# vovw/algonauts-2025

Measured on AMD Instinct MI355X. Metric: TRs/sec trimodal encode to 1000 parcels, higher is better.
Workload: dtype bf16; 1 GPU; trimodal encode, precomputed bf16 feats, per GPU B=64 sequences (4 subjects x R=16) x T=1024, L*D=4096 per modality, hidden 3072, 8 layers, V=1000 parcels, n_output_timesteps=1024; forward only; global_batch=64, seq_len=1024, parallelism=dp1

## Files before the change

algonauts-2025_amd/csrc/attention.hip:

```cpp
#include "attn_common.h"
#include "attn_acc_regs.h"

namespace {

template <int DH>
struct AttnCfg {
  static constexpr int NSUB = DH <= 64 ? 4 : (DH <= 128 ? 2 : 1);
  static constexpr int KS = DH / 32;
  static constexpr int DT = DH / 16;
  static constexpr int ROWB = DH * 2;
  static constexpr int KV = 32 * NSUB;
  static constexpr int TILE_BYTES = KV * ROWB;
  static constexpr int CHUNKS = DH / 8;
  static constexpr int WAVES = 8;
  static constexpr int PIECES = KV * CHUNKS / 64;
  static constexpr int PPW = (PIECES + WAVES - 1) / WAVES;
  static constexpr int SWZ_MASK = (CHUNKS % 16 == 0) ? 15 : 7;
  static constexpr int NBUF = DH >= 192 ? 3 : 2;
  static constexpr int SMEM = NBUF * 2 * TILE_BYTES;
  static_assert(DH % 64 == 0, "dim_head must be a multiple of 64");
};

template <int DH>
__device__ __forceinline__ int swz_chunk(int chunk, int row) {
  constexpr int MASK = AttnCfg<DH>::SWZ_MASK;
  return (chunk & ~MASK) | ((chunk ^ ((row & 7) << 1)) & MASK);
}


template <int DH, int CAUSAL, int RELKEY>
__global__ __launch_bounds__(512, 2) void attn_fwd_kernel(const AttnArgs a) {
  using C = AttnCfg<DH>;
  extern __shared__ __attribute__((aligned(16))) char smem[];
  const int tid = threadIdx.x, lane = tid & 63;
  const int wave = __builtin_amdgcn_readfirstlane(tid >> 6);
  const int fq = lane >> 4, l15 = lane & 15;

  const int T = a.T;
  const float scale_log2e = a.scale_log2e;
  const int xcd = blockIdx.x & 7, slot = blockIdx.x >> 3;
  const int qb = slot % a.qblocks;
  const int pair = (slot / a.qblocks) * 8 + xcd;
  if (pair >= a.n_bh) return;
  const int h = pair % a.heads_q;
  const int b = pair / a.heads_q;
  const int hk = h / a.group;
  const int64_t ld = a.ld_kv;
  const unsigned short* qbase = a.q + (int64_t)b * T * a.ld_q + (int64_t)h * DH;
  const unsigned short* kbase = a.k + (int64_t)b * T * ld + (int64_t)hk * DH;
  const unsigned short* vbase = a.v + (int64_t)b * T * ld + (int64_t)hk * DH;

  const int q0 = qb * 128 + wave * 16;
  const int qrow = (q0 + l15 < T) ? q0 + l15 : T - 1;
  bf16x8_t qf[C::KS];
#pragma unroll
  for (int ks = 0; ks < C::KS; ++ks) qf[ks] = *(const bf16x8_t*)(qbase + (int64_t)qrow * a.ld_q + ks * 32 + fq * 8);

  int st_row[C::PPW], st_src[C::PPW], st_off[C::PPW];
#pragma unroll
  for (int i = 0; i < C::PPW; ++i) {
    const int p = (wave + C::WAVES * i) * 64 + lane;
    st_row[i] = p / C::CHUNKS;
    st_src[i] = swz_chunk<DH>(p % C::CHUNKS, st_row[i]) * 8;
    st_off[i] = st_row[i] * (int)ld + st_src[i];
  }
  auto stage = [&](int buf, int key0) {
    char* kdst = smem + buf * 2 * C::TILE_BYTES;
    const unsigned short* kb = kbase + (int64_t)key0 * ld;
    const unsigned short* vb = vbase + (int64_t)key0 * ld;
    const bool full = key0 + C::KV <= T;
#pragma unroll
    for (int i = 0; i < C::PPW; ++i) {
      const int piece = wave + C::WAVES * i;
      if (piece < C::PIECES) {
        int off = st_off[i];
        if (!full) {
          const int row = (key0 + st_row[i] < T) ? st_row[i] : T - 1 - key0;
          off = row * (int)ld + st_src[i];
        }
        glds16(kb + off, lds_addr(kdst + piece * 1024));
        glds16(vb + off, lds_addr(kdst + C::TILE_BYTES + piece * 1024));
      }
    }
  };

  constexpr int SEG = C::SWZ_MASK + 1;
  constexpr int KRD = SEG / 4;
  int k_rd[KRD];
#pragma unroll
  for (int i = 0; i < KRD; ++i) k_rd[i] = l15 * C::ROWB + swz_chunk<DH>(4 * i + fq, l15) * 16;
  const int tq = l15 >> 2, tp = l15 & 3;
  constexpr int VRD = SEG / 2;
  int v_rd[VRD];
#pragma unroll
  for (int i = 0; i < VRD; ++i) {
    const int row = 4 * fq + tq;
    v_rd[i] = row * C::ROWB + swz_chunk<DH>(2 * i + (tp >> 1), row) * 16 + (tp & 1) * 8;
  }

  f32x4_t o[C::DT];
#pragma unroll
  for (int dt = 0; dt < C::DT; ++dt) o[dt] = f32x4_t{0.f, 0.f, 0.f, 0.f};
  float m_run = -INFINITY, l_run = 0.f;
  constexpr bool LSUM_MFMA = C::NSUB > 1;
  f32x4_t lacc = {0.f, 0.f, 0.f, 0.f};
  bf16x8_t ones;
#pragma unroll
  for (int e = 0; e < 8; ++e) ones[e] = (short)0x3F80;

  int kv_end = T;
  if (CAUSAL) { const int last_q = qb * 128 + 127; kv_end = (last_q + 1 < T) ? last_q + 1 : T; }
  const int ntiles = (kv_end + C::KV - 1) / C::KV;
  int my_glds = 0;
#pragma unroll
  for (int i = 0; i < C::PPW; ++i) my_glds += (wave + C::WAVES * i < C::PIECES) ? 2 : 0;
  auto wait_keep_one_tile = [&]() {
    if (my_glds >= 6) asm volatile("s_waitcnt vmcnt(6)" ::: "memory");
    else if (my_glds == 4) asm volatile("s_waitcnt vmcnt(4)" ::: "memory");
    else if (my_glds == 2) asm volatile("s_waitcnt vmcnt(2)" ::: "memory");
    else asm volatile("s_waitcnt vmcnt(0)" ::: "memory");
  };
  static_assert(C::NBUF == 2 || C::PPW <= 3, "wait_keep_one_tile handles up to 6 loads per tile and wave");
  stage(0, 0);
  if (C::NBUF == 3 && ntiles > 1) { stage(1, C::KV); wait_keep_one_tile(); } else { asm volatile("s_waitcnt vmcnt(0)" ::: "memory"); }
  __syncthreads();

  for (int t = 0; t < ntiles; ++t) {
    const int cur = t % C::NBUF;
    if (C::NBUF == 2 && t + 1 < ntiles) stage(cur ^ 1, (t + 1) * C::KV);
    const char* kt = smem + cur * 2 * C::TILE_BYTES;
    const char* vt = kt + C::TILE_BYTES;
    if (!CAUSAL || t * C::KV <= q0 + 15) {

    float sv[C::NSUB][8];
    float pmax = -INFINITY;
    const int lim = CAUSAL ? ((q0 + l15 + 1 < T) ? q0 + l15 + 1 : T) : T;
#pragma unroll
    for (int u = 0; u < C::NSUB; ++u) {
      const int sub_key0 = t * C::KV + u * 32;
      if (sub_key0 >= T || (CAUSAL && sub_key0 > q0 + 15)) {
#pragma unroll
        for (int j = 0; j < 8; ++j) sv[u][j] = -INFINITY;
        continue;
      }
      f32x4_t s0 = {0.f, 0.f, 0.f, 0.f}, s1 = {0.f, 0.f, 0.f, 0.f};
#pragma unroll
      for (int ks = 0; ks < C::KS; ++ks) {
        const int off = k_rd[ks % KRD] + (ks / KRD) * SEG * 16 + u * 32 * C::ROWB;
        const bf16x8_t ka = *(const bf16x8_t*)(kt + off);
        const bf16x8_t kb2 = *(const bf16x8_t*)(kt + off + 16 * C::ROWB);
        s0 = __builtin_amdgcn_mfma_f32_16x16x32_bf16(ka, qf[ks], s0, 0, 0, 0);
        s1 = __builtin_amdgcn_mfma_f32_16x16x32_bf16(kb2, qf[ks], s1, 0, 0, 0);
      }
      const int key_base = sub_key0 + 4 * fq;
      if (RELKEY) {
        const float* qrow_e = a.qe + ((int64_t)b * T + qrow) * a.ld_qe + h * a.qe_stride_h + a.rel_left;
#pragma unroll
        for (int r = 0; r < 4; ++r) {
          int d0 = key_base + r - qrow, d1 = key_base + 16 + r - qrow;
          d0 = d0 < -a.rel_left ? -a.rel_left : (d0 > a.rel_right ? a.rel_right : d0);
          d1 = d1 < -a.rel_left ? -a.rel_left : (d1 > a.rel_right ? a.rel_right : d1);
          s0[r] += qrow_e[d0];
          s1[r] += qrow_e[d1];
        }
      }
      const bool edge = sub_key0 + 32 > T || (CAUSAL && sub_key0 + 31 > q0);
      if (edge) {
#pragma unroll
        for (int r = 0; r < 4; ++r) {
          sv[u][r] = (key_base + r < lim) ? s0[r] : -INFINITY;
          sv[u][4 + r] = (key_base + 16 + r < lim) ? s1[r] : -INFINITY;
        }
      } else {
#pragma unroll
        for (int r = 0; r < 4; ++r) { sv[u][r] = s0[r]; sv[u][4 + r] = s1[r]; }
      }
      pmax = fmaxf(pmax, fmaxf(sv[u][0], sv[u][4]));
#pragma unroll
      for (int r = 1; r < 4; ++r) pmax = max3f(pmax, sv[u][r], sv[u][4 + r]);
    }
    pmax = fmaxf(pmax, __shfl_xor(pmax, 16, 64));
    pmax = fmaxf(pmax, __shfl_xor(pmax, 32, 64));
    pmax *= scale_log2e;
    if (!__all(pmax - m_run <= 8.0f)) {
      const float m_new = fmaxf(m_run, pmax);
      const float alpha = __builtin_amdgcn_exp2f(m_run - m_new);
      m_run = m_new;
      l_run *= alpha;
      if (LSUM_MFMA) {
#pragma unroll
        for (int r = 0; r < 4; ++r) lacc[r] *= alpha;
      }
#pragma unroll
      for (int dt = 0; dt < C::DT; ++dt)
#pragma unroll
        for (int r = 0; r < 4; ++r) o[dt][r] *= alpha;
    }
    bf16x8_t pf[C::NSUB];
    float psum = 0.f;
#pragma unroll
    for (int u = 0; u < C::NSUB; ++u)
#pragma unroll
      for (int j = 0; j < 8; ++j) {
        const float p = __builtin_amdgcn_exp2f(fmaf(sv[u][j], scale_log2e, -m_run));
        if (!LSUM_MFMA) psum += p;
        pf[u][j] = (short)f32_to_bf16(p);
      }
    l_run += psum;

#pragma unroll
    for (int u = 0; u < C::NSUB; ++u) {
      const int sub_key0 = t * C::KV + u * 32;
      if (sub_key0 >= T || (CAUSAL && sub_key0 > q0 + 15)) continue;
      if (LSUM_MFMA) lacc = __builtin_amdgcn_mfma_f32_16x16x32_bf16(ones, pf[u], lacc, 0, 0, 0);
#pragma unroll
      for (int dt = 0; dt < C::DT; ++dt) {
        const int off = v_rd[dt % VRD] + (dt / VRD) * SEG * 16 + u * 32 * C::ROWB;
        const s16x4_t lo = __builtin_amdgcn_ds_read_tr16_b64_v4i16((__attribute__((address_space(3))) s16x4_t*)(vt + off));
        const s16x4_t hi =
            __builtin_amdgcn_ds_read_tr16_b64_v4i16((__attribute__((address_space(3))) s16x4_t*)(vt + off + 16 * C::ROWB));
        bf16x8_t vf;
#pragma unroll
        for (int e = 0; e < 4; ++e) { vf[e] = lo[e]; vf[4 + e] = hi[e]; }
        o[dt] = __builtin_amdgcn_mfma_f32_16x16x32_bf16(vf, pf[u], o[dt], 0, 0, 0);
      }
    }
    }
    if (C::NBUF == 3) {
      asm volatile("s_waitcnt lgkmcnt(0)" ::: "memory");
      if (t + 2 < ntiles) { stage((t + 2) % C::NBUF, (t + 2) * C::KV); wait_keep_one_tile(); }
      else { asm volatile("s_waitcnt vmcnt(0)" ::: "memory"); }
      __builtin_amdgcn_s_barrier();
    } else {
      asm volatile("s_waitcnt vmcnt(0)" ::: "memory");
      __syncthreads();
    }
  }

  float l_tot;
  if (LSUM_MFMA) {
    l_tot = lacc[0];
  } else {
    l_tot = l_run + __shfl_xor(l_run, 16, 64);
    l_tot += __shfl_xor(l_tot, 32, 64);
  }
  const float inv = 1.0f / l_tot;
  const int q = q0 + l15;
  if (q < T) {
    unsigned short* orow = a.out + ((int64_t)b * T + q) * a.ld_out + (int64_t)h * DH + 4 * fq;
#pragma unroll
    for (int dt = 0; dt < C::DT; ++dt) {
      u16x4_t pk;
#pragma unroll
      for (int e = 0; e < 4; ++e) pk[e] = f32_to_bf16(o[dt][e] * inv);
      *(u16x4_t*)(orow + 16 * dt) = pk;
    }
  }
}


struct WideCfg {
  static constexpr int DH = 384, KS = 24, DT = 12, ROWB = 768, KV = 32, CHUNKS = 48;
  static constexpr int TILE_BYTES = KV * ROWB;
  static constexpr int WAVES = 4, PPW = 6;
  static constexpr int K_SLOTS = 2, V_SLOTS = 4;
  static constexpr int V_BASE = K_SLOTS * TILE_BYTES;
  static constexpr int SMEM = (K_SLOTS + V_SLOTS) * TILE_BYTES;
  static constexpr int DEPTH = 6;
};

__device__ __forceinline__ int swz_wide(int chunk, int row) {
  return (chunk & ~15) | ((chunk ^ (((row & 3) << 2) | ((row >> 2) & 3))) & 15);
}


__device__ __forceinline__ void mfma_s_first(f32x16_t& acc, const bf16x8_t& a, const bf16x8_t& b) {
  asm volatile("v_mfma_f32_32x32x16_bf16 %0, %1, %2, 0" : "=&v"(acc) : "v"(a), "v"(b));
}
__device__ __forceinline__ void mfma_s(f32x16_t& acc, const bf16x8_t& a, const bf16x8_t& b) {
  asm volatile("v_mfma_f32_32x32x16_bf16 %0, %1, %2, %0" : "+v"(acc) : "v"(a), "v"(b));
}


__global__ __launch_bounds__(256, 1) void attn_fwd_wide384_kernel(const AttnArgs a) {
  using C = WideCfg;
  extern __shared__ __attribute__((aligned(16))) char smem[];
  const int tid = threadIdx.x, lane = tid & 63;
  const int wave = __builtin_amdgcn_readfirstlane(tid >> 6);
  const int r31 = lane & 31, h = lane >> 5;

  const int T = a.T;
  const float scale_log2e = a.scale_log2e;
  const int xcd = blockIdx.x & 7, slot = blockIdx.x >> 3;
  const int qb = slot % a.qblocks;
  const int pair = (slot / a.qblocks) * 8 + xcd;
  if (pair >= a.n_bh) return;
  const int hd = pair % a.heads_q;
  const int b = pair / a.heads_q;
  const int hk = hd / a.group;
  const int64_t ld = a.ld_kv;
  const unsigned short* qbase = a.q + (int64_t)b * T * a.ld_q + (int64_t)hd * C::DH;
  const unsigned short* kbase = a.k + (int64_t)b * T * ld + (int64_t)hk * C::DH;
  const unsigned short* vbase = a.v + (int64_t)b * T * ld + (int64_t)hk * C::DH;

  const int q0 = qb * 128 + wave * 32;
  const int qrow = (q0 + r31 < T) ? q0 + r31 : T - 1;
  bf16x8_t qf[C::KS];
#pragma unroll
  for (int ks = 0; ks < C::KS; ++ks) qf[ks] = *(const bf16x8_t*)(qbase + (int64_t)qrow * a.ld_q + ks * 16 + h * 8);
  if (a.q_cos) {
    const int half = a.q_rot_dim >> 1;
    const float* cr = a.q_cos + (int64_t)qrow * half;
    const float* sr = a.q_sin + (int64_t)qrow * half;
#pragma unroll
    for (int ks = 0; ks < C::KS; ++ks) {
      const int d0 = ks * 16 + h * 8;
      if (d0 < a.q_rot_dim) {
        const float4 c4 = *(const float4*)(cr + (d0 >> 1)), s4 = *(const float4*)(sr + (d0 >> 1));
        const float cs[4] = {c4.x, c4.y, c4.z, c4.w}, sn[4] = {s4.x, s4.y, s4.z, s4.w};
#pragma unroll
        for (int pp = 0; pp < 4; ++pp) {
          const float qa = bf16_to_f32((unsigned short)qf[ks][2 * pp]), qb = bf16_to_f32((unsigned short)qf[ks][2 * pp + 1]);
          qf[ks][2 * pp] = (short)f32_to_bf16(qa * cs[pp] - qb * sn[pp]);
          qf[ks][2 * pp + 1] = (short)f32_to_bf16(qb * cs[pp] + qa * sn[pp]);
        }
      }
    }
  }

  int st_row[C::PPW], st_src[C::PPW], st_off[C::PPW];
#pragma unroll
  for (int i = 0; i < C::PPW; ++i) {
    const int p = (wave + C::WAVES * i) * 64 + lane;
    st_row[i] = p / C::CHUNKS;
    st_src[i] = swz_wide(p % C::CHUNKS, st_row[i]) * 8;
    st_off[i] = st_row[i] * (int)ld + st_src[i];
  }
  const unsigned lds0_u = __builtin_amdgcn_readfirstlane(lds_addr(smem));
  auto stage_piece = [&](int which, int slot, int key0, int i) {
    const char* sbase = (const char*)((which ? vbase : kbase) + (int64_t)key0 * ld);
    const int piece = wave + C::WAVES * i;
    unsigned voff = (unsigned)st_off[i] * 2u;
    if (key0 + C::KV > T) {
      const int row = (key0 + st_row[i] < T) ? st_row[i] : T - 1 - key0;
      voff = (unsigned)(row * (int)ld + st_src[i]) * 2u;
    }
    const unsigned dst = lds0_u + (which ? C::V_BASE : 0) + slot * C::TILE_BYTES + piece * 1024;
    asm volatile("s_mov_b32 m0, %0\n\ts_nop 0\n\tglobal_load_lds_dwordx4 %1, %2" : : "s"(dst), "v"(voff), "s"(sbase) : "memory");
  };
  auto stage = [&](int which, int slot, int key0) {
#pragma unroll
    for (int i = 0; i < C::PPW; ++i) stage_piece(which, slot, key0, i);
  };

  int kb_off[8];
#pragma unroll
  for (int i = 0; i < 8; ++i) kb_off[i] = r31 * C::ROWB + swz_wide(2 * i + h, r31) * 16;
  const int tq = (lane & 15) >> 2, tp = lane & 3, g1 = (lane >> 4) & 1;
  int vb_off[4][2];
#pragma unroll
  for (int i = 0; i < 4; ++i)
#pragma unroll
    for (int lh = 0; lh < 2; ++lh) {
      const int row = 4 * h + tq + 8 * lh;
      vb_off[i][lh] = C::V_BASE + row * C::ROWB + swz_wide(4 * i + 2 * g1 + (tp >> 1), row) * 16 + (tp & 1) * 8;
    }
  auto ld_k = [&](const int (&ka)[8], int ks) -> bf16x8_t {
    return *(const bf16x8_t*)(smem + ka[ks & 7] + (ks >> 3) * 256);
  };
  auto ld_v = [&](const int (&va)[4][2], int i) -> bf16x8_t {
    const int s = i / C::DT, dt = i % C::DT;
    const int imm = (dt >> 2) * 256 + s * 16 * C::ROWB;
    const s16x4_t lo = __builtin_amdgcn_ds_read_tr16_b64_v4i16((__attribute__((address_space(3))) s16x4_t*)(smem + va[dt & 3][0] + imm));
    const s16x4_t hi = __builtin_amdgcn_ds_read_tr16_b64_v4i16((__attribute__((address_space(3))) s16x4_t*)(smem + va[dt & 3][1] + imm));
    bf16x8_t vf;
#pragma unroll
    for (int e = 0; e < 4; ++e) { vf[e] = lo[e]; vf[4 + e] = hi[e]; }
    return vf;
  };

  static_for<0, C::DT>([&](auto dt) { AccTile<decltype(dt)::value>::zero(); });
  float m_run = -INFINITY, l_run = 0.f;

  const int ntiles = (T + C::KV - 1) / C::KV;
  stage(0, 0, 0); stage(1, 0, 0);
  if (ntiles > 1) { stage(0, 1, C::KV); stage(1, 1, C::KV); asm volatile("s_waitcnt vmcnt(12)" ::: "memory"); }
  else { asm volatile("s_waitcnt vmcnt(0)" ::: "memory"); }
  __builtin_amdgcn_s_barrier();

  bf16x8_t kf[C::KS], vf[2 * C::DT];
  int ka[8], va[4][2];
#pragma unroll
  for (int i = 0; i < 8; ++i) ka[i] = kb_off[i];
#pragma unroll
  for (int i = 0; i < 4; ++i) { va[i][0] = vb_off[i][0]; va[i][1] = vb_off[i][1]; }
#pragma unroll
  for (int d = 0; d < C::DEPTH; ++d) kf[d] = ld_k(ka, d);

#ifdef TRIBE_ATTN_STAMPS
  unsigned long long ts0 = 0, ts1 = 0, ts2 = 0, ts3 = 0, ts4 = 0, ts5 = 0;
  unsigned long long stamp_acc[5] = {0, 0, 0, 0, 0};
#endif
  int vcur = 0;
  for (int t = 0; t < ntiles; ++t) {
    ATTN_STAMP(ts0);
    const bool more = t + 2 < ntiles;
    const int vnext2 = (vcur + 2) & 3;

    f32x16_t s;
#pragma unroll
    for (int ks = 0; ks < C::KS; ++ks) {
      if (ks + C::DEPTH < C::KS) kf[ks + C::DEPTH] = ld_k(ka, ks + C::DEPTH);
      else vf[ks + C::DEPTH - C::KS] = ld_v(va, ks + C::DEPTH - C::KS);
      if (ks % 4 == 1) { if (more) stage_piece(1, vnext2, (t + 2) * C::KV, ks / 4); }
      __builtin_amdgcn_sched_barrier(0);
      if (ks == 0) mfma_s_first(s, kf[ks], qf[ks]);
      else mfma_s(s, kf[ks], qf[ks]);
      __builtin_amdgcn_sched_barrier(0);
    }
    asm volatile("s_nop 11" : "+v"(s));
    ATTN_STAMP(ts1);

    if ((t + 1) * C::KV > T) {
#pragma unroll
      for (int r = 0; r < 16; ++r)
        if (t * C::KV + (r & 3) + 8 * (r >> 2) + 4 * h >= T) s[r] = -INFINITY;
    }
    float pmax = max3f(s[0], s[1], s[2]);
#pragma unroll
    for (int r = 3; r < 15; r += 2) pmax = max3f(pmax, s[r], s[r + 1]);
    pmax = fmaxf(pmax, s[15]);
    pmax = pair_max(pmax) * scale_log2e;
    if (!__all(pmax - m_run <= 8.0f)) {
      const float m_new = fmaxf(m_run, pmax);
      const float alpha = __builtin_amdgcn_exp2f(m_run - m_new);
      m_run = m_new;
      l_run *= alpha;
      if (t > 0) {
        asm volatile("s_nop 15\n\ts_nop 7" ::: "memory");
        static_for<0, C::DT>([&](auto dt) { AccTile<decltype(dt)::value>::scale(alpha); });
        asm volatile("s_nop 7" ::: "memory");
      }
    }
    bf16x8_t pf[2];
    float psum = 0.f;
#pragma unroll
    for (int r = 0; r < 16; ++r) {
      const float p = __builtin_amdgcn_exp2f(fmaf(s[r], scale_log2e, -m_run));
      psum += p;
      pf[r >> 3][r & 7] = (short)f32_to_bf16(p);
    }
    l_run += psum;

    ATTN_STAMP(ts2);
    if (more) asm volatile("s_waitcnt vmcnt(6)" ::: "memory");
    else asm volatile("s_waitcnt vmcnt(0)" ::: "memory");
    ATTN_STAMP(ts3);
    __builtin_amdgcn_s_barrier();
    ATTN_STAMP(ts4);
    const int kslot = t & 1;
    const int kstep = kslot ? -C::TILE_BYTES : C::TILE_BYTES;
#pragma unroll
    for (int i = 0; i < 8; ++i) asm volatile("v_add_u32 %0, %1, %0" : "+v"(ka[i]) : "s"(kstep));
    asm volatile("s_nop 1" : "+v"(pf[0]), "+v"(pf[1]));

    static_for<0, 2 * C::DT>([&](auto ic) {
      constexpr int i = decltype(ic)::value;
      if constexpr (i + C::DEPTH < 2 * C::DT) vf[i + C::DEPTH] = ld_v(va, i + C::DEPTH);
      else kf[i + C::DEPTH - 2 * C::DT] = ld_k(ka, i + C::DEPTH - 2 * C::DT);
      if constexpr (i % 4 == 1) { if (more) stage_piece(0, kslot, (t + 2) * C::KV, i / 4); }
      __builtin_amdgcn_sched_barrier(0);
      AccTile<i % C::DT>::mfma(vf[i], pf[i / C::DT]);
      __builtin_amdgcn_sched_barrier(0);
    });
    const int vstep = (vcur == 3) ? -3 * C::TILE_BYTES : C::TILE_BYTES;
#pragma unroll
    for (int i = 0; i < 4; ++i) {
      asm volatile("v_add_u32 %0, %1, %0" : "+v"(va[i][0]) : "s"(vstep));
      asm volatile("v_add_u32 %0, %1, %0" : "+v"(va[i][1]) : "s"(vstep));
    }
    vcur = (vcur + 1) & 3;
    ATTN_STAMP(ts5);
    ATTN_STAMP_ADD(0, ts0, ts1); ATTN_STAMP_ADD(1, ts1, ts2); ATTN_STAMP_ADD(2, ts2, ts3); ATTN_STAMP_ADD(3, ts3, ts4); ATTN_STAMP_ADD(4, ts4, ts5);
  }
#ifdef TRIBE_ATTN_STAMPS
  if (a.qe != nullptr && lane == 0) {
    unsigned long long* dbg = (unsigned long long*)a.qe + ((size_t)blockIdx.x * 4 + wave) * 8;
    for (int i = 0; i < 5; ++i) dbg[i] = stamp_acc[i];
    dbg[5] = (unsigned long long)ntiles;
  }
#endif

  asm volatile("s_nop 15\n\ts_nop 7" ::: "memory");
  const float l_tot = pair_sum(l_run);
  const float inv = 1.0f / l_tot;
  const int q = q0 + r31;
  if (a.lse != nullptr && h == 0 && q < T) a.lse[((int64_t)b * a.heads_q + hd) * T + q] = m_run + __builtin_amdgcn_logf(l_tot);
  unsigned short* orow = a.out + ((int64_t)b * T + (q < T ? q : T - 1)) * a.ld_out + (int64_t)hd * C::DH + 4 * h;
  static_for<0, C::DT>([&](auto dtc) {
    constexpr int dt = decltype(dtc)::value;
    float ov[16];
    AccTile<dt>::read(ov);
    if (q < T) {
#pragma unroll
      for (int g = 0; g < 4; ++g) {
        u16x4_t pk;
#pragma unroll
        for (int e = 0; e < 4; ++e) pk[e] = f32_to_bf16(ov[4 * g + e] * inv);
        *(u16x4_t*)(orow + 32 * dt + 8 * g) = pk;
      }
    }
  });
}

struct KSplitCfg {
  static constexpr int DH = 384, ROWB = 768, KV = 32, CHUNKS = 48;
  static constexpr int KS = 12, NT = 6, Q_AGPR = 8;
  static constexpr int TILE_BYTES = KV * ROWB;
  static constexpr int WAVES = 8, PPW = 6;
  static constexpr int SLOTS = 5;
  static constexpr int X_BASE = SLOTS * TILE_BYTES;
  static constexpr int SMEM = X_BASE + WAVES * 4096;
  static constexpr int DEPTH = 4;
};

__global__ __launch_bounds__(512, 2) void attn_fwd_ksplit384_kernel(const AttnArgs a) {
  using C = KSplitCfg;
  extern __shared__ __attribute__((aligned(16))) char smem[];
  const int tid = threadIdx.x, lane = tid & 63;
  const int wave = __builtin_amdgcn_readfirstlane(tid >> 6);
  const int qj = wave & 3, c = wave >> 2;
  const int r31 = lane & 31, h = lane >> 5;

  const int T = a.T;
  const float scale_log2e = a.scale_log2e;
  const int xcd = blockIdx.x & 7, slot = blockIdx.x >> 3;
  const int qb = slot % a.qblocks;
  const int pair = (slot / a.qblocks) * 8 + xcd;
  if (pair >= a.n_bh) return;
  const int hd = pair % a.heads_q;
  const int b = pair / a.heads_q;
  const int hk = hd / a.group;
  const int64_t ld = a.ld_kv;
  const unsigned short* qbase = a.q + (int64_t)b * T * a.ld_q + (int64_t)hd * C::DH;
  const unsigned short* kbase = a.k + (int64_t)b * T * ld + (int64_t)hk * C::DH;
  const unsigned short* vbase = a.v + (int64_t)b * T * ld + (int64_t)hk * C::DH;

  const int q0 = qb * 128 + qj * 32;
  const int qrow = (q0 + r31 < T) ? q0 + r31 : T - 1;
  bf16x8_t qv[C::KS - C::Q_AGPR];
  static_for<0, C::KS>([&](auto kc) {
    constexpr int k = decltype(kc)::value;
    const int ksg = 8 * (k >> 2) + 4 * c + (k & 3);
    const bf16x8_t qfrag = *(const bf16x8_t*)(qbase + (int64_t)qrow * a.ld_q + ksg * 16 + h * 8);
    if constexpr (k < C::Q_AGPR) QFrag<k>::set(qfrag);
    else qv[k - C::Q_AGPR] = qfrag;
  });
  static_for<0, C::NT>([&](auto n) { AccTile<decltype(n)::value>::zero(); });
  asm volatile("s_nop 7" ::: "memory");

  int st_off[C::PPW];
#pragma unroll
  for (int i = 0; i < C::PPW; ++i) {
    const int p = (qj + 4 * i) * 64 + lane;
    st_off[i] = (p / C::CHUNKS) * (int)ld + swz_wide(p % C::CHUNKS, p / C::CHUNKS) * 8;
  }
  const unsigned short* my_base = c ? vbase : kbase;
  auto stage_piece = [&](int slot_i, int key0, int i) {
    const unsigned short* src = my_base + (int64_t)key0 * ld;
    const int piece = qj + 4 * i;
    int off = st_off[i];
    if (key0 + C::KV > T) {
      const int p = piece * 64 + lane;
      const int row0 = p / C::CHUNKS;
      const int row = (key0 + row0 < T) ? row0 : T - 1 - key0;
      off = row * (int)ld + swz_wide(p % C::CHUNKS, row0) * 8;
    }
    glds16(src + off, lds_addr(smem) + slot_i * C::TILE_BYTES + piece * 1024);
  };

  int ka[4];
#pragma unroll
  for (int i = 0; i < 4; ++i) ka[i] = r31 * C::ROWB + swz_wide(8 * c + 2 * i + h, r31) * 16;
  const int tq = (lane & 15) >> 2, tp = lane & 3, g1 = (lane >> 4) & 1;
  int va[2][2];
#pragma unroll
  for (int e = 0; e < 2; ++e)
#pragma unroll
    for (int lh = 0; lh < 2; ++lh) {
      const int row = 4 * h + tq + 8 * lh;
      va[e][lh] = C::TILE_BYTES + row * C::ROWB + swz_wide(4 * (2 * c + e) + 2 * g1 + (tp >> 1), row) * 16 + (tp & 1) * 8;
    }
  auto ld_k = [&](int k) -> bf16x8_t { return *(const bf16x8_t*)(smem + ka[k & 3] + (k >> 2) * 256); };
  auto ld_v = [&](int i) -> bf16x8_t {
    const int sk = i / C::NT, n = i % C::NT;
    const int imm = (n >> 1) * 256 + sk * 16 * C::ROWB;
    const s16x4_t lo = __builtin_amdgcn_ds_read_tr16_b64_v4i16((__attribute__((address_space(3))) s16x4_t*)(smem + va[n & 1][0] + imm));
    const s16x4_t hi = __builtin_amdgcn_ds_read_tr16_b64_v4i16((__attribute__((address_space(3))) s16x4_t*)(smem + va[n & 1][1] + imm));
    bf16x8_t vf;
#pragma unroll
    for (int e = 0; e < 4; ++e) { vf[e] = lo[e]; vf[4 + e] = hi[e]; }
    return vf;
  };
  const int x_mine = C::X_BASE + wave * 4096 + lane * 16, x_peer = C::X_BASE + (wave ^ 4) * 4096 + lane * 16;

  float m_run = -INFINITY, l_run = 0.f;
  const int ntiles = (T + C::KV - 1) / C::KV;
  auto stage_half = [&](int hh) {
    if ((hh & 1) != c) return;
#pragma unroll
    for (int i = 0; i < C::PPW; ++i) stage_piece(hh % C::SLOTS, (hh >> 1) * C::KV, i);
  };
  const int nhalf = 2 * ntiles;
  for (int hh = 0; hh < C::SLOTS && hh < nhalf; ++hh) stage_half(hh);
  if (c == 0) {
    if (ntiles >= 3) asm volatile("s_waitcnt vmcnt(12)" ::: "memory");
    else if (ntiles == 2) asm volatile("s_waitcnt vmcnt(6)" ::: "memory");
    else asm volatile("s_waitcnt vmcnt(0)" ::: "memory");
  }
  __builtin_amdgcn_s_barrier();

  bf16x8_t kf[C::KS], vf[2 * C::NT];
#pragma unroll
  for (int d = 0; d < C::DEPTH; ++d) kf[d] = ld_k(d);

  int kslot = 0, vslot = 1;
  for (int t = 0; t < ntiles; ++t) {
    f32x16_t s;
    static_for<0, C::KS>([&](auto kc) {
      constexpr int k = decltype(kc)::value;
#ifndef TRIBE_ATTN_DMA_ONLY
      if constexpr (k + C::DEPTH < C::KS) kf[k + C::DEPTH] = ld_k(k + C::DEPTH);
#endif
      if constexpr (k % 2 == 1) { if (c == 0 && t >= 1 && t + 2 < ntiles) stage_piece((2 * t + 4) % C::SLOTS, (t + 2) * C::KV, k / 2); }
      __builtin_amdgcn_sched_barrier(0);
#ifndef TRIBE_ATTN_DMA_ONLY
      if constexpr (k == 0) QFrag<k>::mfma_first(s, kf[k]);
      else if constexpr (k < C::Q_AGPR) QFrag<k>::mfma(s, kf[k]);
      else mfma_s(s, kf[k], qv[k - C::Q_AGPR]);
#else
      if constexpr (k == 0) { for (int r = 0; r < 16; ++r) s[r] = (float)r31; }
#endif
      __builtin_amdgcn_sched_barrier(0);
    });
    asm volatile("s_nop 11" : "+v"(s));
#pragma unroll
    for (int q4 = 0; q4 < 4; ++q4) *(f32x4_t*)(smem + x_mine + q4 * 1024) = f32x4_t{s[4 * q4], s[4 * q4 + 1], s[4 * q4 + 2], s[4 * q4 + 3]};
    if (c == 0 ? (t + 2 < ntiles) : (t + 1 < ntiles)) asm volatile("s_waitcnt vmcnt(6) lgkmcnt(0)" ::: "memory");
    else asm volatile("s_waitcnt vmcnt(0) lgkmcnt(0)" ::: "memory");
    __builtin_amdgcn_s_barrier();
#pragma unroll
    for (int d = 0; d < C::DEPTH; ++d) vf[d] = ld_v(d);
#pragma unroll
    for (int q4 = 0; q4 < 4; ++q4) {
      const f32x4_t o4 = *(const f32x4_t*)(smem + x_peer + q4 * 1024);
#pragma unroll
      for (int e = 0; e < 4; ++e) s[4 * q4 + e] += o4[e];
    }

    if ((t + 1) * C::KV > T) {
#pragma unroll
      for (int r = 0; r < 16; ++r)
        if (t * C::KV + (r & 3) + 8 * (r >> 2) + 4 * h >= T) s[r] = -INFINITY;
    }
    float pmax = max3f(s[0], s[1], s[2]);
#pragma unroll
    for (int r = 3; r < 15; r += 2) pmax = max3f(pmax, s[r], s[r + 1]);
    pmax = fmaxf(pmax, s[15]);
    pmax = pair_max(pmax) * scale_log2e;
    if (!__all(pmax - m_run <= 8.0f)) {
      const float m_new = fmaxf(m_run, pmax);
      const float alpha = __builtin_amdgcn_exp2f(m_run - m_new);
      m_run = m_new;
      l_run *= alpha;
      if (t > 0) {
        asm volatile("s_nop 15\n\ts_nop 7" ::: "memory");
        static_for<0, C::NT>([&](auto n) { AccTile<decltype(n)::value>::scale(alpha); });
        asm volatile("s_nop 7" ::: "memory");
      }
    }
    bf16x8_t pf[2];
    float psum = 0.f;
#pragma unroll
    for (int r = 0; r < 16; ++r) {
      const float p = __builtin_amdgcn_exp2f(fmaf(s[r], scale_log2e, -m_run));
      psum += p;
      pf[r >> 3][r & 7] = (short)f32_to_bf16(p);
    }
    l_run += psum;

    const int knext = kslot + 2 >= C::SLOTS ? kslot + 2 - C::SLOTS : kslot + 2;
    const int kstep = (knext - kslot) * C::TILE_BYTES;
#pragma unroll
    for (int i = 0; i < 4; ++i) asm volatile("v_add_u32 %0, %1, %0" : "+v"(ka[i]) : "s"(kstep));
    asm volatile("s_nop 1" : "+v"(pf[0]), "+v"(pf[1]));

    static_for<0, 2 * C::NT>([&](auto ic) {
      constexpr int i = decltype(ic)::value;
#ifndef TRIBE_ATTN_DMA_ONLY
      if constexpr (i + C::DEPTH < 2 * C::NT) vf[i + C::DEPTH] = ld_v(i + C::DEPTH);
      else kf[i + C::DEPTH - 2 * C::NT] = ld_k(i + C::DEPTH - 2 * C::NT);
#endif
      if constexpr (i % 2 == 1) { if (c == 1 && t + 2 < ntiles) stage_piece(kslot, (t + 2) * C::KV, i / 2); }
      __builtin_amdgcn_sched_barrier(0);
#ifndef TRIBE_ATTN_DMA_ONLY
      AccTile<i % C::NT>::mfma(vf[i], pf[i / C::NT]);
#endif
      __builtin_amdgcn_sched_barrier(0);
    });
    const int vnext = vslot + 2 >= C::SLOTS ? vslot + 2 - C::SLOTS : vslot + 2;
    const int vstep = (vnext - vslot) * C::TILE_BYTES;
#pragma unroll
    for (int e = 0; e < 2; ++e) {
      asm volatile("v_add_u32 %0, %1, %0" : "+v"(va[e][0]) : "s"(vstep));
      asm volatile("v_add_u32 %0, %1, %0" : "+v"(va[e][1]) : "s"(vstep));
    }
    kslot = knext;
    vslot = vnext;
    __builtin_amdgcn_s_barrier();
  }

  asm volatile("s_nop 15\n\ts_nop 7" ::: "memory");
  const float inv = 1.0f / pair_sum(l_run);
  const int q = q0 + r31;
  unsigned short* orow = a.out + ((int64_t)b * T + (q < T ? q : T - 1)) * a.ld_out + (int64_t)hd * C::DH + 4 * h + 64 * c;
  static_for<0, C::NT>([&](auto nc) {
    constexpr int n = decltype(nc)::value;
    float ov[16];
    AccTile<n>::read(ov);
    if (q < T) {
#pragma unroll
      for (int g = 0; g < 4; ++g) {
        u16x4_t pk;
#pragma unroll
        for (int e = 0; e < 4; ++e) pk[e] = f32_to_bf16(ov[4 * g + e] * inv);
        *(u16x4_t*)(orow + 128 * (n >> 1) + 32 * (n & 1) + 8 * g) = pk;
      }
    }
  });
}

int launch_attn_ksplit384(const AttnArgs& a, int64_t B, hipStream_t s) {
  using C = KSplitCfg;
  static bool attr_done = false;
  if (!attr_done) {
    (void)hipFuncSetAttribute((const void*)attn_fwd_ksplit384_kernel, hipFuncAttributeMaxDynamicSharedMemorySize, C::SMEM);
    attr_done = true;
  }
  const int64_t nblocks = (B * a.heads_q + 7) / 8 * 8 * a.qblocks;
  if (nblocks >= (1ll << 31)) { tribe_set_error("tribe_attention_fwd: grid too large"); return -1; }
  if ((int64_t)a.T * a.ld_kv >= (1ll << 31)) { tribe_set_error("tribe_attention_fwd: sequence too long for 32-bit offsets"); return -1; }
  hipLaunchKernelGGL(attn_fwd_ksplit384_kernel, dim3((unsigned)nblocks), dim3(512), C::SMEM, s, a);
  TRIBE_LAUNCH_CHECK();
  return 0;
}

int launch_attn_wide384(const AttnArgs& a, int64_t B, hipStream_t s) {
  using C = WideCfg;
  static bool attr_done = false;
  if (!attr_done) {
    (void)hipFuncSetAttribute((const void*)attn_fwd_wide384_kernel, hipFuncAttributeMaxDynamicSharedMemorySize, C::SMEM);
    attr_done = true;
  }
  const int64_t nblocks = (B * a.heads_q + 7) / 8 * 8 * a.qblocks;
  if (nblocks >= (1ll << 31)) { tribe_set_error("tribe_attention_fwd: grid too large"); return -1; }
  if ((int64_t)a.T * a.ld_kv >= (1ll << 31)) { tribe_set_error("tribe_attention_fwd: sequence too long for 32-bit offsets"); return -1; }
  hipLaunchKernelGGL(attn_fwd_wide384_kernel, dim3((unsigned)nblocks), dim3(256), C::SMEM, s, a);
  TRIBE_LAUNCH_CHECK();
  return 0;
}

template <int DH, int CAUSAL, int RELKEY>
int launch_attn(const AttnArgs& a, int64_t B, hipStream_t s) {
  using C = AttnCfg<DH>;
  static bool attr_done = false;
  if (!attr_done) {
    (void)hipFuncSetAttribute((const void*)attn_fwd_kernel<DH, CAUSAL, RELKEY>, hipFuncAttributeMaxDynamicSharedMemorySize, C::SMEM);
    attr_done = true;
  }
  const int64_t nblocks = (B * a.heads_q + 7) / 8 * 8 * a.qblocks;
  if (nblocks >= (1ll << 31)) { tribe_set_error("tribe_attention_fwd: grid too large"); return -1; }
  if ((int64_t)a.T * a.ld_kv >= (1ll << 31)) { tribe_set_error("tribe_attention_fwd: sequence too long for 32-bit offsets"); return -1; }
  hipLaunchKernelGGL((attn_fwd_kernel<DH, CAUSAL, RELKEY>), dim3((unsigned)nblocks), dim3(512), C::SMEM, s, a);
  TRIBE_LAUNCH_CHECK();
  return 0;
}

}
int tribe_internal_attn_d64_launch(const void* args, int64_t B, int relkey, int variant, hipStream_t s);
namespace {

int g_attn_d64_variant = 0;
int g_attn_wide384 = 1;

template <int DH>
int launch_attn_dh(const AttnArgs& a, int64_t B, int causal, hipStream_t s) {
  if (DH == 384 && !causal && g_attn_wide384 == 1) return launch_attn_wide384(a, B, s);
  if (DH == 384 && !causal && g_attn_wide384 == 2) return launch_attn_ksplit384(a, B, s);
  return causal ? launch_attn<DH, 1, 0>(a, B, s) : launch_attn<DH, 0, 0>(a, B, s);
}

}

void tribe_internal_attention_set_wide384(int on) { g_attn_wide384 = on; }
void tribe_internal_attention_set_d64_variant(int v) { g_attn_d64_variant = v; }

int tribe_internal_attention_fused_supported(int dim_head) {
  return dim_head == 64 || dim_head == 128 || dim_head == 192 || dim_head == 384;
}

static int attention_dispatch_impl(const tribe_attention_desc* d, const float* q_cos, const float* q_sin, int q_rot_dim, void* stream);
static int attention_dispatch(const tribe_attention_desc* d, const float* q_cos, const float* q_sin, int q_rot_dim, void* stream) {
  const double flops = d ? 4.0 * (double)d->T * (double)d->dim_head * (double)d->T * (double)d->heads_q * (double)d->B * (d->causal ? 0.5 : 1.0) : 0.0;
  const int slot = tribe_internal_prof_before(TRIBE_ROLE_ATTENTION, flops, (hipStream_t)stream);
  const int rc = attention_dispatch_impl(d, q_cos, q_sin, q_rot_dim, stream);
  tribe_internal_prof_after(slot, (hipStream_t)stream);
  return rc;
}
static int attention_dispatch_impl(const tribe_attention_desc* d, const float* q_cos, const float* q_sin, int q_rot_dim, void* stream) {
  TRIBE_REQUIRE(d && d->q && d->k && d->v && d->out, "tribe_attention_fwd_ex: null pointer");
  TRIBE_REQUIRE(d->B > 0 && d->T > 0 && d->heads_q > 0 && d->heads_kv > 0 && d->heads_q % d->heads_kv == 0,
                "tribe_attention_fwd_ex: bad shape (B=%lld T=%lld heads %d/%d)", (long long)d->B, (long long)d->T, d->heads_q, d->heads_kv);
  TRIBE_REQUIRE(tribe_internal_attention_fused_supported(d->dim_head), "tribe_attention_fwd_ex: dim_head=%d not in {64,128,192,384}",
                d->dim_head);
  TRIBE_REQUIRE(d->ld_k == d->ld_v, "tribe_attention_fwd_ex: k and v must share their row stride");
  TRIBE_REQUIRE(d->ld_q % 8 == 0 && d->ld_k % 8 == 0 && d->ld_out % 4 == 0 && ((uintptr_t)d->q % 16) == 0 && ((uintptr_t)d->k % 16) == 0 &&
                    ((uintptr_t)d->v % 16) == 0 && ((uintptr_t)d->out % 8) == 0,
                "tribe_attention_fwd_ex: operands must be 16-byte aligned with row strides that are multiples of 8");
  AttnArgs a;
  a.q = d->q; a.k = d->k; a.v = d->v; a.out = d->out;
  a.ld_q = d->ld_q; a.ld_kv = d->ld_k; a.ld_out = d->ld_out;
  a.T = (int)d->T; a.heads_q = d->heads_q; a.group = d->heads_q / d->heads_kv;
  a.scale_log2e = d->scale * 1.4426950408889634f;
  a.qblocks = (int)((d->T + 127) / 128);
  a.n_bh = (int)(d->B * d->heads_q);
  a.qe = d->rel_qe; a.ld_qe = d->ld_rel_qe; a.qe_stride_h = d->rel_stride_h; a.rel_left = d->rel_left; a.rel_right = d->rel_right;
  a.q_cos = q_cos; a.q_sin = q_sin; a.q_rot_dim = q_rot_dim;
  a.lse = d->lse;
  TRIBE_REQUIRE(!d->lse || (tribe_attention_lse_supported(d->dim_head, d->causal) && !d->rel_qe),
                "tribe_attention_fwd_ex: the log-sum-exp output exists for dim_head 384, bidirectional, default mode only");
  hipStream_t s = (hipStream_t)stream;
#ifdef TRIBE_ATTN_STAMPS
  if (d->rel_qe && d->dim_head == 384) return launch_attn_dh<384>(a, d->B, d->causal, s);
  if (d->rel_qe && d->dim_head == 64 && d->rel_left < 0) return tribe_internal_attn_d64_launch(&a, d->B, 0, g_attn_d64_variant, s);
#endif
  if (d->rel_qe) {
    TRIBE_REQUIRE(d->dim_head == 64 && !d->causal, "tribe_attention_fwd_ex: the relative_key bias is built for dim_head 64, non-causal");
    TRIBE_REQUIRE(d->rel_left >= 0 && d->rel_right >= 0 && d->rel_stride_h >= d->rel_left + d->rel_right + 1 &&
                      d->ld_rel_qe >= (int64_t)d->heads_q * d->rel_stride_h,
                  "tribe_attention_fwd_ex: bad relative_key table geometry");
    return g_attn_wide384 ? tribe_internal_attn_d64_launch(&a, d->B, 1, g_attn_d64_variant, s) : launch_attn<64, 0, 1>(a, d->B, s);
  }
  switch (d->dim_head) {
    case 64: return (!d->causal && g_attn_wide384) ? tribe_internal_attn_d64_launch(&a, d->B, 0, g_attn_d64_variant, s) : launch_attn_dh<64>(a, d->B, d->causal, s);
    case 128: return launch_attn_dh<128>(a, d->B, d->causal, s);
    case 192: return launch_attn_dh<192>(a, d->B, d->causal, s);
    default: return launch_attn_dh<384>(a, d->B, d->causal, s);
  }
}

extern "C" int tribe_attention_fwd_ex(const tribe_attention_desc* d, void* stream) { return attention_dispatch(d, nullptr, nullptr, 0, stream); }

extern "C" int tribe_attention_lse_supported(int32_t dim_head, int32_t causal) { return dim_head == 384 && !causal && g_attn_wide384 == 1; }

int tribe_internal_attention_rotates_q(int dim_head) { return dim_head == 384 && g_attn_wide384 == 1; }

static tribe_attention_desc fused_desc(const uint16_t* qkv, int64_t B, int64_t T, int heads, int dim_head, float scale, uint16_t* out) {
  const int64_t inner = (int64_t)heads * dim_head;
  tribe_attention_desc d;
  d.q = qkv; d.k = qkv + inner; d.v = qkv + 2 * inner;
  d.ld_q = d.ld_k = d.ld_v = 3 * inner;
  d.out = out; d.ld_out = inner;
  d.B = B; d.T = T; d.heads_q = heads; d.heads_kv = heads; d.dim_head = dim_head; d.causal = 0; d.scale = scale;
  d.rel_qe = nullptr; d.ld_rel_qe = 0; d.rel_stride_h = 0; d.rel_left = d.rel_right = 0;
  d.lse = nullptr;
  return d;
}

int tribe_internal_attention_fused_qrot(const uint16_t* qkv, int64_t B, int64_t T, int heads, int dim_head, float scale, uint16_t* out,
                                        const float* cos_tab, const float* sin_tab, int rot_dim, hipStream_t s) {
  TRIBE_REQUIRE(tribe_internal_attention_rotates_q(dim_head) && cos_tab && sin_tab && rot_dim > 0 && rot_dim % 16 == 0 && rot_dim <= dim_head,
                "tribe_internal_attention_fused_qrot: unsupported configuration");
  const tribe_attention_desc d = fused_desc(qkv, B, T, heads, dim_head, scale, out);
  return attention_dispatch(&d, cos_tab, sin_tab, rot_dim, (void*)s);
}

int tribe_internal_attention_fused(const uint16_t* qkv, int64_t B, int64_t T, int heads, int dim_head, float scale, uint16_t* out,
                                   hipStream_t s) {
  const tribe_attention_desc d = fused_desc(qkv, B, T, heads, dim_head, scale, out);
  return attention_dispatch(&d, nullptr, nullptr, 0, (void*)s);
}
```

Measured before the change: 630,200 TRs/s.

## Overlap K/V prefetch with Q rotary load, batch rotary loads, widen output stores

The wide dim-384 attention kernel now issues the first two K/V tile stages before loading Q and applying rotary, so the global-to-LDS copies overlap the Q prologue. The rotary cos/sin loads are batched, with a template count of batches that picks one or two passes depending on the rotary width, and scheduling barriers are used to group the loads before the math. The epilogue packs bf16 outputs and uses permlane32_swap so each lane writes 16-byte stores instead of 8-byte ones, which requires a 16-byte aligned output and is now checked. Debug timestamp plumbing is also added under a compile flag.

Measured after the change: 631,900 TRs/s (median of 6 runs). About the same (+0.3%).

```diff
diff --git a/algonauts-2025_amd/csrc/attention.hip b/algonauts-2025_amd/csrc/attention.hip
--- a/algonauts-2025_amd/csrc/attention.hip
+++ b/algonauts-2025_amd/csrc/attention.hip
@@ -282,6 +282,7 @@
 }
 
 
+template <int QROT_BATCHES>
 __global__ __launch_bounds__(256, 1) void attn_fwd_wide384_kernel(const AttnArgs a) {
   using C = WideCfg;
   extern __shared__ __attribute__((aligned(16))) char smem[];
@@ -302,31 +303,10 @@
   const unsigned short* qbase = a.q + (int64_t)b * T * a.ld_q + (int64_t)hd * C::DH;
   const unsigned short* kbase = a.k + (int64_t)b * T * ld + (int64_t)hk * C::DH;
   const unsigned short* vbase = a.v + (int64_t)b * T * ld + (int64_t)hk * C::DH;
-
-  const int q0 = qb * 128 + wave * 32;
-  const int qrow = (q0 + r31 < T) ? q0 + r31 : T - 1;
-  bf16x8_t qf[C::KS];
-#pragma unroll
-  for (int ks = 0; ks < C::KS; ++ks) qf[ks] = *(const bf16x8_t*)(qbase + (int64_t)qrow * a.ld_q + ks * 16 + h * 8);
-  if (a.q_cos) {
-    const int half = a.q_rot_dim >> 1;
-    const float* cr = a.q_cos + (int64_t)qrow * half;
-    const float* sr = a.q_sin + (int64_t)qrow * half;
-#pragma unroll
-    for (int ks = 0; ks < C::KS; ++ks) {
-      const int d0 = ks * 16 + h * 8;
-      if (d0 < a.q_rot_dim) {
-        const float4 c4 = *(const float4*)(cr + (d0 >> 1)), s4 = *(const float4*)(sr + (d0 >> 1));
-        const float cs[4] = {c4.x, c4.y, c4.z, c4.w}, sn[4] = {s4.x, s4.y, s4.z, s4.w};
-#pragma unroll
-        for (int pp = 0; pp < 4; ++pp) {
-          const float qa = bf16_to_f32((unsigned short)qf[ks][2 * pp]), qb = bf16_to_f32((unsigned short)qf[ks][2 * pp + 1]);
-          qf[ks][2 * pp] = (short)f32_to_bf16(qa * cs[pp] - qb * sn[pp]);
-          qf[ks][2 * pp + 1] = (short)f32_to_bf16(qb * cs[pp] + qa * sn[pp]);
-        }
-      }
-    }
-  }
+#ifdef TRIBE_ATTN_STAMPS
+  unsigned long long tp0 = 0, tp1 = 0, te0 = 0, te1 = 0;
+#endif
+  ATTN_STAMP(tp0);
 
   int st_row[C::PPW], st_src[C::PPW], st_off[C::PPW];
 #pragma unroll
@@ -352,6 +332,61 @@
 #pragma unroll
     for (int i = 0; i < C::PPW; ++i) stage_piece(which, slot, key0, i);
   };
+
+  const int ntiles = (T + C::KV - 1) / C::KV;
+
+  stage(0, 0, 0); stage(1, 0, 0);
+  if (ntiles > 1) { stage(0, 1, C::KV); stage(1, 1, C::KV); }
+
+  const int q0 = qb * 128 + wave * 32;
+  const int qrow = (q0 + r31 < T) ? q0 + r31 : T - 1;
+  bf16x8_t qf[C::KS];
+#pragma unroll
+  for (int ks = 0; ks < C::KS; ++ks) qf[ks] = *(const bf16x8_t*)(qbase + (int64_t)qrow * a.ld_q + ks * 16 + h * 8);
+  if constexpr (QROT_BATCHES > 0) {
+    const int half = a.q_rot_dim >> 1, nrot = a.q_rot_dim >> 4;
+    const float* cr = a.q_cos + (int64_t)qrow * half + h * 4;
+    const float* sr = a.q_sin + (int64_t)qrow * half + h * 4;
+    constexpr int RB = C::KS / 2;
+#pragma unroll
+    for (int bt = 0; bt < QROT_BATCHES; ++bt) {
+      f32x4_t c4[RB], s4[RB];
+#pragma unroll
+      for (int j = 0; j < RB; ++j) {
+        const int ks = bt * RB + j, pair0 = ks < nrot ? ks * 8 : 0;
+        c4[j] = *(const f32x4_t*)(cr + pair0);
+        s4[j] = *(const f32x4_t*)(sr + pair0);
+      }
+      __builtin_amdgcn_sched_barrier(0);
+      static_assert(RB == 12, "the operand list below names 12 k-steps");
+      asm volatile("" : "+v"(c4[0]), "+v"(c4[1]), "+v"(c4[2]), "+v"(c4[3]), "+v"(c4[4]), "+v"(c4[5]), "+v"(c4[6]), "+v"(c4[7]), "+v"(c4[8]),
+                        "+v"(c4[9]), "+v"(c4[10]), "+v"(c4[11]), "+v"(s4[0]), "+v"(s4[1]), "+v"(s4[2]), "+v"(s4[3]), "+v"(s4[4]), "+v"(s4[5]),
+                        "+v"(s4[6]), "+v"(s4[7]), "+v"(s4[8]), "+v"(s4[9]), "+v"(s4[10]), "+v"(s4[11]));
+      __builtin_amdgcn_sched_barrier(0);
+#pragma unroll
+      for (int j = 0; j < RB; ++j) {
+        const int ks = bt * RB + j;
+        const float cs[4] = {c4[j][0], c4[j][1], c4[j][2], c4[j][3]}, sn[4] = {s4[j][0], s4[j][1], s4[j][2], s4[j][3]};
+        bf16x8_t rq;
+#pragma unroll
+        for (int pp = 0; pp < 4; ++pp) {
+          const float qa = bf16_to_f32((unsigned short)qf[ks][2 * pp]), qb = bf16_to_f32((unsigned short)qf[ks][2 * pp + 1]);
+          rq[2 * pp] = (short)f32_to_bf16(qa * cs[pp] - qb * sn[pp]);
+          rq[2 * pp + 1] = (short)f32_to_bf16(qb * cs[pp] + qa * sn[pp]);
+        }
+        qf[ks] = ks < nrot ? rq : qf[ks];
+        asm volatile("" : "+v"(qf[ks]));
+      }
+      __builtin_amdgcn_sched_barrier(0);
+    }
+  } else {
+    __builtin_amdgcn_sched_barrier(0);
+    asm volatile("" : "+v"(qf[C::KS - 1]));
+  }
+  asm volatile("s_waitcnt vmcnt(0)" ::: "memory");
+  __builtin_amdgcn_s_barrier();
+  ATTN_STAMP(tp1);
+  __builtin_amdgcn_sched_barrier(0);
 
   int kb_off[8];
 #pragma unroll
@@ -381,12 +416,6 @@
 
   static_for<0, C::DT>([&](auto dt) { AccTile<decltype(dt)::value>::zero(); });
   float m_run = -INFINITY, l_run = 0.f;
-
-  const int ntiles = (T + C::KV - 1) / C::KV;
-  stage(0, 0, 0); stage(1, 0, 0);
-  if (ntiles > 1) { stage(0, 1, C::KV); stage(1, 1, C::KV); asm volatile("s_waitcnt vmcnt(12)" ::: "memory"); }
-  else { asm volatile("s_waitcnt vmcnt(0)" ::: "memory"); }
-  __builtin_amdgcn_s_barrier();
 
   bf16x8_t kf[C::KS], vf[2 * C::DT];
   int ka[8], va[4][2];
@@ -483,34 +512,43 @@
     ATTN_STAMP(ts5);
     ATTN_STAMP_ADD(0, ts0, ts1); ATTN_STAMP_ADD(1, ts1, ts2); ATTN_STAMP_ADD(2, ts2, ts3); ATTN_STAMP_ADD(3, ts3, ts4); ATTN_STAMP_ADD(4, ts4, ts5);
   }
+  ATTN_STAMP(te0);
+
+  asm volatile("s_nop 15\n\ts_nop 7" ::: "memory");
+  const float l_tot = pair_sum(l_run);
+  const float inv = 1.0f / l_tot;
+  const int q = q0 + r31;
+  if (a.lse != nullptr && h == 0 && q < T) a.lse[((int64_t)b * a.heads_q + hd) * T + q] = m_run + __builtin_amdgcn_logf(l_tot);
+  unsigned short* orow = a.out + ((int64_t)b * T + (q < T ? q : T - 1)) * a.ld_out + (int64_t)hd * C::DH + 8 * h;
+  static_for<0, C::DT>([&](auto dtc) {
+    constexpr int dt = decltype(dtc)::value;
+    float ov[16];
+    AccTile<dt>::read(ov);
+    uint2 pk[4];
+#pragma unroll
+    for (int g = 0; g < 4; ++g) {
+      u16x4_t p4;
+#pragma unroll
+      for (int e = 0; e < 4; ++e) p4[e] = f32_to_bf16(ov[4 * g + e] * inv);
+      pk[g] = __builtin_bit_cast(uint2, p4);
+    }
+#pragma unroll
+    for (int g = 0; g < 4; g += 2) {
+      const auto sx = __builtin_amdgcn_permlane32_swap(pk[g].x, pk[g + 1].x, false, false);
+      const auto sy = __builtin_amdgcn_permlane32_swap(pk[g].y, pk[g + 1].y, false, false);
+      if (q < T) *(uint4*)(orow + 32 * dt + 8 * g) = make_uint4(sx[0], sy[0], sx[1], sy[1]);
+    }
+  });
+  ATTN_STAMP(te1);
 #ifdef TRIBE_ATTN_STAMPS
   if (a.qe != nullptr && lane == 0) {
     unsigned long long* dbg = (unsigned long long*)a.qe + ((size_t)blockIdx.x * 4 + wave) * 8;
     for (int i = 0; i < 5; ++i) dbg[i] = stamp_acc[i];
     dbg[5] = (unsigned long long)ntiles;
+    dbg[6] = tp1 - tp0;
+    dbg[7] = te1 - te0;
   }
 #endif
-
-  asm volatile("s_nop 15\n\ts_nop 7" ::: "memory");
-  const float l_tot = pair_sum(l_run);
-  const float inv = 1.0f / l_tot;
-  const int q = q0 + r31;
-  if (a.lse != nullptr && h == 0 && q < T) a.lse[((int64_t)b * a.heads_q + hd) * T + q] = m_run + __builtin_amdgcn_logf(l_tot);
-  unsigned short* orow = a.out + ((int64_t)b * T + (q < T ? q : T - 1)) * a.ld_out + (int64_t)hd * C::DH + 4 * h;
-  static_for<0, C::DT>([&](auto dtc) {
-    constexpr int dt = decltype(dtc)::value;
-    float ov[16];
-    AccTile<dt>::read(ov);
-    if (q < T) {
-#pragma unroll
-      for (int g = 0; g < 4; ++g) {
-        u16x4_t pk;
-#pragma unroll
-        for (int e = 0; e < 4; ++e) pk[e] = f32_to_bf16(ov[4 * g + e] * inv);
-        *(u16x4_t*)(orow + 32 * dt + 8 * g) = pk;
-      }
-    }
-  });
 }
 
 struct KSplitCfg {
@@ -755,19 +793,28 @@
   return 0;
 }
 
-int launch_attn_wide384(const AttnArgs& a, int64_t B, hipStream_t s) {
+template <int QROT_BATCHES>
+int launch_attn_wide384_q(const AttnArgs& a, int64_t nblocks, hipStream_t s) {
   using C = WideCfg;
   static bool attr_done = false;
   if (!attr_done) {
-    (void)hipFuncSetAttribute((const void*)attn_fwd_wide384_kernel, hipFuncAttributeMaxDynamicSharedMemorySize, C::SMEM);
+    (void)hipFuncSetAttribute((const void*)attn_fwd_wide384_kernel<QROT_BATCHES>, hipFuncAttributeMaxDynamicSharedMemorySize, C::SMEM);
     attr_done = true;
   }
+  hipLaunchKernelGGL(attn_fwd_wide384_kernel<QROT_BATCHES>, dim3((unsigned)nblocks), dim3(256), C::SMEM, s, a);
+  TRIBE_LAUNCH_CHECK();
+  return 0;
+}
+
+int launch_attn_wide384(const AttnArgs& a, int64_t B, hipStream_t s) {
   const int64_t nblocks = (B * a.heads_q + 7) / 8 * 8 * a.qblocks;
   if (nblocks >= (1ll << 31)) { tribe_set_error("tribe_attention_fwd: grid too large"); return -1; }
   if ((int64_t)a.T * a.ld_kv >= (1ll << 31)) { tribe_set_error("tribe_attention_fwd: sequence too long for 32-bit offsets"); return -1; }
-  hipLaunchKernelGGL(attn_fwd_wide384_kernel, dim3((unsigned)nblocks), dim3(256), C::SMEM, s, a);
-  TRIBE_LAUNCH_CHECK();
-  return 0;
+  TRIBE_REQUIRE(a.ld_out % 8 == 0 && ((uintptr_t)a.out % 16) == 0,
+                "tribe_attention_fwd: dim_head 384 needs a 16-byte aligned output with a row stride that is a multiple of 8 (ld_out=%lld)",
+                (long long)a.ld_out);
+  if (!a.q_cos) return launch_attn_wide384_q<0>(a, nblocks, s);
+  return 16 * (WideCfg::KS / 2) >= a.q_rot_dim ? launch_attn_wide384_q<1>(a, nblocks, s) : launch_attn_wide384_q<2>(a, nblocks, s);
 }
 
 template <int DH, int CAUSAL, int RELKEY>
@@ -817,6 +864,10 @@
   tribe_internal_prof_after(slot, (hipStream_t)stream);
   return rc;
 }
+#ifdef TRIBE_ATTN_STAMPS
+static const float* g_attn_stamp_buf = nullptr;
+extern "C" void tribe_debug_attn_stamp_buffer(void* p) { g_attn_stamp_buf = (const float*)p; }
+#endif
 static int attention_dispatch_impl(const tribe_attention_desc* d, const float* q_cos, const float* q_sin, int q_rot_dim, void* stream) {
   TRIBE_REQUIRE(d && d->q && d->k && d->v && d->out, "tribe_attention_fwd_ex: null pointer");
   TRIBE_REQUIRE(d->B > 0 && d->T > 0 && d->heads_q > 0 && d->heads_kv > 0 && d->heads_q % d->heads_kv == 0,
@@ -842,6 +893,7 @@
   hipStream_t s = (hipStream_t)stream;
 #ifdef TRIBE_ATTN_STAMPS
   if (d->rel_qe && d->dim_head == 384) return launch_attn_dh<384>(a, d->B, d->causal, s);
+  if (!d->rel_qe && g_attn_stamp_buf && d->dim_head == 384) { a.qe = g_attn_stamp_buf; return launch_attn_dh<384>(a, d->B, d->causal, s); }
   if (d->rel_qe && d->dim_head == 64 && d->rel_left < 0) return tribe_internal_attn_d64_launch(&a, d->B, 0, g_attn_d64_variant, s);
 #endif
   if (d->rel_qe) {
```
